# SharperJBCA/COMAPreduce

Measured on AMD Instinct MI355X. Metric: TOD samples x channels / s (L1 -> L2 reduction), higher is better.
Workload: dtype f32 in, f64 accumulate

## Files before the change

### comapreduce_amd/csrc/comap_internal.h

```cpp
#pragma once
#include <hip/hip_runtime.h>
#include <cstdint>
#include <string>
#include <vector>

#include "../../include/comap_hip.h"

struct comap_ctx {
    int device = 0;
    hipStream_t stream = nullptr;
    std::string err;
    void *scratch = nullptr;
    size_t scratch_bytes = 0;
};

#define COMAP_CHECK(ctx, expr)                                                         \
    do {                                                                               \
        hipError_t _e = (expr);                                                        \
        if (_e != hipSuccess) {                                                        \
            (ctx)->err = std::string(#expr) + ": " + hipGetErrorString(_e);            \
            return -2;                                                                 \
        }                                                                              \
    } while (0)

// ... 102 lines not shown
    int32_t wmL = 0;
    size_t wm_smem = 0;
    int32_t *slo = nullptr;
    int32_t *redo = nullptr;
    void *krange = nullptr;
    void *temp = nullptr;
    size_t temp_bytes = 0;
    int64_t numax = 0;
    bool blocksort = true;
    hipEvent_t plan_ev = nullptr;
    hipStream_t alloc_stream = nullptr;
    hipStream_t run_stream = nullptr;
};

int comap_median_plan(comap_ctx *ctx, MedPlan *mp, const std::vector<MedJob> &jobs, int32_t w);
void comap_median_plan_free(MedPlan *mp);
int comap_median_run(comap_ctx *ctx, MedPlan *mp, hipStream_t stream);
inline int comap_median_run(comap_ctx *ctx, MedPlan *mp) { return comap_median_run(ctx, mp, ctx->stream); }
int comap_median_replay(comap_ctx *ctx, const std::vector<MedJob> &jobs, int32_t w, hipStream_t st);

struct comap_l1_plan {
    comap_ctx *ctx = nullptr;
    int32_t F = 0, S = 0, U = 0;
    int64_t T = 0;
    const float *tod = nullptr;
    const double *el = nullptr;
    std::vector<int32_t> units_h;
    int32_t *units = nullptr;
    int32_t *tiles = nullptr;
    int64_t n_tiles = 0;
    int32_t *tiles_b = nullptr;
    int64_t *gaps = nullptr;
    int64_t n_gaps = 0, max_gap = 0;
    static constexpr int kMaxGroups = 4;
    int32_t ngroups = 0;
    int32_t grp_u0[kMaxGroups + 1] = {0};
    int64_t grp_tile0[kMaxGroups + 1] = {0};
    int64_t grpb_tile0[kMaxGroups + 1] = {0};
    MedPlan medg[kMaxGroups];
    hipStream_t side = nullptr;
    hipEvent_t ev_b[kMaxGroups] = {}, ev_m[kMaxGroups] = {};
    double *airmass = nullptr;
    double *unit_sums = nullptr;
    double *mom = nullptr;
    int32_t *nan_count = nullptr;
    bool moments_valid = false;
    bool moments_pending = false;
    bool prefetched = false;
    int32_t *nan_host = nullptr;
    hipEvent_t mom_event = nullptr;
    double *alpha = nullptr;
    double *nf = nullptr;
    double *bsum = nullptr;
    double *mb = nullptr;
    double *mf = nullptr;
    double *ssum = nullptr;
    double *sdm = nullptr;
    double *sgb = nullptr;
    double *pdot = nullptr;
    double *pgate = nullptr;
    int32_t *needc = nullptr;
    bool regress_legacy = false;
    double *gw = nullptr;
    int32_t *gmode = nullptr;
    double *kap = nullptr;
    double *dsum = nullptr;
    double *xreg = nullptr;
    double *dG = nullptr;
    int32_t *rowbad = nullptr;
    int32_t nan_total = 0;
    bool filled = false;
    int64_t *nanpos = nullptr;
    int64_t nanpos_cap = 0;
    int64_t *nanpos_n = nullptr;
// ... 32 lines not shown
```

### comapreduce_amd/csrc/l1_kernels.hip

```cpp
#include "comap_internal.h"

#include <algorithm>
#include <cfloat>
#include <cmath>
#include <cstdlib>
#include <cstring>
#include <type_traits>
#include <utility>

using namespace comap;

#ifndef COMAP_GROUPS
#define COMAP_GROUPS 1
#endif

typedef float f32x4u __attribute__((ext_vector_type(4), aligned(4)));
__device__ __forceinline__ f32x4u ld4(const float *p)
{
    return __builtin_nontemporal_load(reinterpret_cast<const f32x4u *>(p));
}

__device__ __forceinline__ double wave_sum(double v)
{
#pragma unroll
    for (int o = 32; o > 0; o >>= 1) v += __shfl_xor(v, o, 64);
    return v;
}

__device__ __forceinline__ int uniform(int v) { return __builtin_amdgcn_readfirstlane(v); }

__device__ __forceinline__ double block_sum256(double v, double *lds4)
{
    v = wave_sum(v);
    const int wid = threadIdx.x >> 6;
    __syncthreads();
    if ((threadIdx.x & 63) == 0) lds4[wid] = v;
    __syncthreads();
    double t = lds4[0] + lds4[1] + lds4[2] + lds4[3];
    return t;
}

__device__ __forceinline__ bool atmos_channel(int c)
{
    return c >= 10 && c < 1014 && !(c >= 510 && c < 515);
}

__device__ __forceinline__ bool median_channel(int c)
// ... 333 lines not shown
{
    const int64_t i = blockIdx.x * (int64_t)blockDim.x + threadIdx.x;
    if (i >= (int64_t)U * kBC) return;
    const int u = (int)(i / kBC);
    const int bc = (int)(i % kBC);
    const int b = bc / kChannels, c = bc % kChannels;
    const int f = units[4 * u], s = units[4 * u + 1];
    const double *q = ubs + 4 * ((int64_t)u * kBands + b);
    const double n = q[0], sa = q[1], saa = q[2];
    double o = NAN, a = NAN;
    if (atmos_channel(c) && n >= 100.0) {
        const double *src = (sel && sel[(int64_t)u * kBands + b]) ? fs_sel : fs;
        const double sd = src[i], sad = src[UC + i];
        const double det = n * saa - sa * sa;
        o = (saa * sd - sa * sad) / det;
        a = (n * sad - sa * sd) / det;
    }
    double *out = fit + (((int64_t)s * F + f) * kBands + b) * 2 * kChannels;
    out[c] = o;
    out[kChannels + c] = a;
}

__global__ void __launch_bounds__(256) k_coef_b(const int32_t *__restrict__ units, const double *__restrict__ us,
                                                const double *__restrict__ mom, int64_t UC,
                                                const double *__restrict__ fit, int F, const float *__restrict__ med,
                                                double *__restrict__ oa,
                                                double *__restrict__ alpha, double *__restrict__ nf,
                                                double *__restrict__ bsum, int32_t *__restrict__ flag)
{
    __shared__ double red[4];
    const int ub = blockIdx.x;
    const int u = ub / kBands, b = ub % kBands;
    const int n = units[4 * u + 3];
    if (ub == 0 && threadIdx.x == 0) *flag = 0;
    const int fu = units[4 * u], su = units[4 * u + 1];
    const double *fo = fit + (((int64_t)su * F + fu) * kBands + b) * 2 * kChannels;
    const double *q = us + 8 * (int64_t)u;
    const double sv = q[3], svv = q[4], n4 = q[5];
    double beta = 0, gamma = 0, cnt = 0;
    for (int c = threadIdx.x; c < kChannels; c += blockDim.x) {
        const int64_t i = (int64_t)u * kBC + b * kChannels + c;
        const double o = med ? (double)med[i] : fo[c], a = med ? 0.0 : fo[kChannels + c];
        oa[2 * i] = o;
        oa[2 * i + 1] = a;
        double rms = NAN;
        if (n4 > 0 && isfinite(o) && isfinite(a)) {
            const double su = mom[2 * UC + i], suu = mom[3 * UC + i], suv = mom[4 * UC + i];
            const double mean = (su - a * sv) / n4;
            double var = (suu - 2.0 * a * suv + a * a * svv) / n4 - mean * mean;
            var = var < 0.0 ? 0.0 : var;
            rms = sqrt(var) / sqrt(2.0) * sqrt(kDnuTau);
        }
        nf[i] = rms;
        double al = 0.0;
        if (median_channel(c)) {
            al = 1.0 / rms;
            if (isfinite(al) && isfinite(o) && isfinite(a)) {
                beta += al * o;
                gamma += al * a;
                cnt += 1.0;
            } else {
                al = 0.0;
            }
        }
        alpha[i] = al;
    }
    beta = block_sum256(beta, red);
// ... 353 lines not shown
        x1 = y1 / u11;
        x0 = (sym - Smm * x1) / Smf;
    } else {
        const double l = Smf / n, u11 = Smm - l * Smf;
        const double y1 = sym - l * sy;
        x1 = y1 / u11;
        x0 = (sy - Smf * x1) / n;
    }
}

__device__ __forceinline__ bool special_row(bool band_on, int c, double al, int32_t rb)
{
    return band_on && median_channel(c) && al != 0.0 && rb > 0;
}

__device__ __forceinline__ double special_y(double al, double o, double a, double x0, double x1, float d, double At,
                                            double mft)
{
    const double m = ((double)d - (o + a * At)) * al;
    return m - (x0 + mft * x1);
}

__device__ __forceinline__ void special_weights(int c, double tsv, double nf, double g, double y0, double &W,
                                                double &Wo)
{
    W = 1.0 / (tsv * tsv);
    if (tsv == 0.0) W = 0.0;
    if (c < 50 || c >= 974 || c == 512 || (c >= 510 && c < 515)) W = 0.0;
    if (isnan(y0 * nf / g)) W = 0.0;
    Wo = W;
    if (isnan(tsv) || isnan(y0 * tsv)) Wo = 0.0;
}

__global__ void __launch_bounds__(256) k_coef_d(const int32_t *__restrict__ units, const double *__restrict__ us,
                                                const double *__restrict__ mom, int64_t UC,
                                                const double *__restrict__ oa,
                                                const double *__restrict__ alpha, const double *__restrict__ nf,
                                                const double *__restrict__ bsum, const double *__restrict__ ss,
                                                double *__restrict__ sdm, const double *__restrict__ tsys0,
                                                const double *__restrict__ gain0, const double *__restrict__ gw,
                                                const int32_t *__restrict__ gmode, int calibrator,
                                                double *__restrict__ kap, double *__restrict__ dsum,
                                                double *__restrict__ xreg, int phase,
                                                int32_t *__restrict__ flag, int32_t *__restrict__ dlist,
                                                int32_t *__restrict__ dcnt, double *__restrict__ dw,
                                                const int32_t *__restrict__ rowbad, const float *__restrict__ tod,
                                                int64_t T, const double *__restrict__ A,
                                                const double *__restrict__ mf, const int32_t *__restrict__ ynf,
                                                const int32_t *__restrict__ ugate, const double *__restrict__ pd,
                                                double *__restrict__ pg, const int32_t *__restrict__ needc)
{
    __shared__ double red[4];
    __shared__ double s_kap[4][kChannels];
    const int ub = blockIdx.x;
    const int u = ub / kBands, b = ub % kBands;
    const int f = units[4 * u];
    const double *q = us + 8 * (int64_t)u;
    const double n = q[0], SA = q[1];
    const double *bs = bsum + 4 * (int64_t)ub;
    const bool band_on = bs[3] > 0;
    const double *sq = ss + 4 * (int64_t)ub;
    const double Smf = sq[0], Smm = sq[1], SAm = sq[2];
    const int gm = gmode[f];
    const bool gate = n >= 5.0 && !(ugate && ugate[u]);
    const bool gain_called = !calibrator && gate;
    const bool zero = gain_called;
    const bool use_dg = gain_called && gm == 0 && !ynf[u];
    const double det = n * Smm - Smf * Smf;
    const bool fused = phase != 0 && band_on && needc[ub] == 0;
    const bool solve = phase != 0 && !fused;
    double pbad = 0.0, pmag = 0.0;
    double acc[12];
#pragma unroll
    for (int k = 0; k < 12; ++k) acc[k] = 0.0;
    for (int c = threadIdx.x; c < kChannels; c += blockDim.x) {
        const int64_t i = (int64_t)u * kBC + b * kChannels + c;
        const double o = oa[2 * i], a = oa[2 * i + 1];
        const double al = alpha[i];
        const double tsv = tsys0[(int64_t)f * kBC + b * kChannels + c];
        const bool zeroed = zero && (gain_masked(c) || isnan(tsv));
        const bool special = special_row(band_on, c, al, rowbad[i]) && !zeroed;
        double fa = 0, fb = 0, fg = 0, fd = 0, x0 = 0, x1 = 0;
        if (band_on && median_channel(c)) {
            if (al != 0.0) {
                const double sdmi = solve ? sdm[i] : 0.0;
                const double sy = al * (mom[i] - n * o - a * SA);
                const double sym = al * (sdmi - o * Smf - a * SAm);
// ... 166 lines not shown
                const int64_t i = kb + rows[k];
                const double y = special_y(alpha[i], oa[2 * i], oa[2 * i + 1], xreg[2 * i], xreg[2 * i + 1],
                                           tod[(fb + rows[k]) * T + t0 + t], a[t], m[t]);
                inf |= isinf(y);
            }
        if (inf) ugate[u] = 1;
        return;
    }
    const double *ds = dsum + 16 * (int64_t)ub;
    const double SW = ds[10], SWo = ds[11];
    double *to = tod_out + ((int64_t)f * kBands + b) * T + t0;
    double *oo = orig_out + ((int64_t)f * kBands + b) * T + t0;
    for (int t = threadIdx.x; t < n; t += blockDim.x) {
        double sr = 0.0, so = 0.0;
        for (int k = 0; k < nr; ++k) {
            const int c = rows[k];
            const int64_t i = kb + c;
            const double y = special_y(alpha[i], oa[2 * i], oa[2 * i + 1], xreg[2 * i], xreg[2 * i + 1],
                                       tod[(fb + c) * T + t0 + t], a[t], m[t]);
            double r = y * nf[i] / gain0[fb + c];
            if (isnan(r)) r = 0.0;
            sr += rw[k] * r;
            double q = y * tsys0[fb + c];
            if (isnan(q)) q = 0.0;
            so += rwo[k] * q;
        }
        to[t] += sr / SW;
        oo[t] += so / SWo;
    }
}

__global__ void __launch_bounds__(256) k_gain_avg(const float *__restrict__ tod, const double *__restrict__ A,
                                                  const int32_t *__restrict__ units, const int32_t *__restrict__ tiles,
                                                  int64_t T, int64_t UC, const double *__restrict__ kap,
                                                  const double *__restrict__ dsum, const double *__restrict__ mf,
                                                  double *__restrict__ tod_out, double *__restrict__ orig_out,
                                                  double *__restrict__ dG_out, const int32_t *__restrict__ flag)
{
    __shared__ double sg[kBands][kTile];
    if (*flag == 0) return;
    const int b = uniform(threadIdx.x >> 6);
    const int lane = threadIdx.x & 63;
    const int u = tiles[2 * blockIdx.x], toff = tiles[2 * blockIdx.x + 1];
    const int f = units[4 * u], t0 = units[4 * u + 2], n = units[4 * u + 3];
    const int r0 = toff + 4 * lane;
    const float *base = tod + (int64_t)(f * kBands + b) * kChannels * T + t0 + r0;
    const int64_t kb = (int64_t)u * kBC + b * kChannels;
    const double *kg = kap + kb, *kr = kap + UC + kb, *ko = kap + 2 * UC + kb;
    double ag[4 * kJ], ar[4 * kJ], ao[4 * kJ];
#pragma unroll
    for (int i = 0; i < 4 * kJ; ++i) ag[i] = ar[i] = ao[i] = 0.0;
    const int nv0 = n - r0;
#pragma unroll 2
    for (int c = 0; c < kChannels; ++c) {
        const double wg = kg[c], wr = kr[c], wo = ko[c];
        if (wg == 0.0 && wr == 0.0 && wo == 0.0) continue;
        double x[4 * kJ];
        load_groups(base + (int64_t)c * T, nv0, x);
#pragma unroll
        for (int i = 0; i < 4 * kJ; ++i) {
            ag[i] = fma(wg, x[i], ag[i]);
            ar[i] = fma(wr, x[i], ar[i]);
            ao[i] = fma(wo, x[i], ao[i]);
        }
    }
    const double *ds = dsum + 16 * ((int64_t)u * kBands + b);
    const double *a = A + (int64_t)f * T + t0 + r0;
    const double *m = mf + (int64_t)(f * kBands + b) * T + t0 + r0;
    double at[4 * kJ], mt[4 * kJ];
#pragma unroll
    for (int g = 0; g < kJ; ++g)
#pragma unroll
        for (int e = 0; e < 4; ++e) {
            const int i = 4 * g + e, o = 256 * g + e;
            const bool ok = o < nv0;
            at[i] = ok ? a[o] : 0.0;
// ... 12 lines not shown
            const int tl = 256 * g + 4 * lane + e;
            const double dG = sg[0][tl] + sg[1][tl] + sg[2][tl] + sg[3][tl];
            const double sr = ar[i] + ds[3] + at[i] * ds[4] + mt[i] * ds[5];
            const double so = ao[i] + ds[6] + at[i] * ds[7] + mt[i] * ds[8];
            to[o] = (sr - dG * ds[9]) / ds[10];
            oo[o] = so / ds[11];
            if (b == 0) dG_out[(int64_t)f * T + t0 + r0 + o] = dG;
        }
}

__device__ __forceinline__ void scan_weight_band(const double *__restrict__ r, int n, double *__restrict__ wo,
                                                 double *red)
{
    const int np = n / 2;
    double s = 0, cnt = 0;
    for (int k = threadIdx.x; k < np; k += blockDim.x) {
        const double d = r[2 * k + 1] - r[2 * k];
        if (!isnan(d)) { s += d; cnt += 1.0; }
    }
    s = block_sum256(s, red);
    cnt = block_sum256(cnt, red);
    const double mean = s / cnt;
    double v = 0;
    for (int k = threadIdx.x; k < np; k += blockDim.x) {
        const double d = r[2 * k + 1] - r[2 * k];
        if (!isnan(d)) v += (d - mean) * (d - mean);
    }
    v = block_sum256(v, red);
    const double rms = sqrt(v / cnt) / sqrt(2.0);
    const double wt = 1.0 / (rms * rms);
    for (int t = threadIdx.x; t < n; t += blockDim.x) wo[t] = wt;
}

__global__ void __launch_bounds__(256) k_scan_weights(const int32_t *__restrict__ units, int64_t T,
                                                      const double *__restrict__ tod_out, double *__restrict__ w_out)
{
    __shared__ double red[4];
    const int ub = blockIdx.x;
    const int u = ub / kBands, b = ub % kBands;
    const int f = units[4 * u], t0 = units[4 * u + 2], n = units[4 * u + 3];
    const int64_t o = (int64_t)(f * kBands + b) * T + t0;
    scan_weight_band(tod_out + o, n, w_out + o, red);
}

__global__ void __launch_bounds__(256) k_finish(const int32_t *__restrict__ units, const int32_t *__restrict__ tiles,
                                                int64_t T, const double *__restrict__ A,
                                                const double *__restrict__ mf, const double *__restrict__ dsum,
                                                double *__restrict__ tod_out, double *__restrict__ orig_out,
                                                double *__restrict__ dG, const int32_t *__restrict__ flag)
{
    if (*flag != 0) return;
    const int u = tiles[2 * blockIdx.x];
    const int f = units[4 * u], t0 = units[4 * u + 2], n = units[4 * u + 3];
    const double *ds = dsum + 16 * (int64_t)u * kBands;
    for (int k = threadIdx.x; k < kTile; k += 256) {
        const int r = tiles[2 * blockIdx.x + 1] + k;
        if (r >= n) break;
        const int64_t t = t0 + r;
        const double a = A[(int64_t)f * T + t];
        double m[kBands], g = dG[(int64_t)f * T + t];
#pragma unroll
        for (int b = 0; b < kBands; ++b) {
            m[b] = mf[(int64_t)(f * kBands + b) * T + t];
            const double *d = ds + 16 * b;
            g += d[0] + a * d[1] + m[b] * d[2];
        }
        dG[(int64_t)f * T + t] = g;
#pragma unroll
        for (int b = 0; b < kBands; ++b) {
            const double *d = ds + 16 * b;
            const int64_t o = (int64_t)(f * kBands + b) * T + t;
            tod_out[o] = (tod_out[o] + d[3] + a * d[4] + m[b] * d[5] - g * d[9]) / d[10];
            orig_out[o] = (orig_out[o] + d[6] + a * d[7] + m[b] * d[8]) / d[11];
        }
    }
}

__global__ void __launch_bounds__(256) k_zero_gaps(const int64_t *__restrict__ gaps, int64_t T, int F,
                                                   double *__restrict__ tod_out, double *__restrict__ orig_out,
                                                   double *__restrict__ w_out)
{
    const int64_t *g = gaps + 3 * (int64_t)blockIdx.y;
    const int64_t f = g[0], t0 = g[1], n = g[2];
    for (int64_t k = blockIdx.x * (int64_t)blockDim.x + threadIdx.x; k < n; k += (int64_t)gridDim.x * blockDim.x) {
#pragma unroll
        for (int b = 0; b < kBands; ++b) {
            const int64_t o = (f * kBands + b) * T + t0 + k;
            tod_out[o] = 0.0;
            orig_out[o] = 0.0;
// ... 203 lines not shown
        }
    }
    std::vector<int32_t> tiles;
    for (int u = 0; u < p->U; ++u)
        for (int t = 0; t < p->units_h[4 * u + 3]; t += kTile) { tiles.push_back(u); tiles.push_back(t); }
    p->n_tiles = (int64_t)tiles.size() / 2;
    std::vector<int32_t> tiles_b;
    std::vector<int64_t> tub(p->U + 1, 0);
    for (int u = 0; u < p->U; ++u) {
        const int shift = (p->T % 32 == 0) ? (p->units_h[4 * u + 2] & 31) : 0;
        for (int t = -shift; t < p->units_h[4 * u + 3]; t += kTile) { tiles_b.push_back(u); tiles_b.push_back(t); }
        tub[u + 1] = (int64_t)tiles_b.size() / 2;
    }
    std::vector<int64_t> gaps;
    {
        std::vector<std::vector<std::pair<int64_t, int64_t>>> cov(p->F);
        for (int u = 0; u < p->U; ++u)
            cov[p->units_h[4 * u]].push_back({p->units_h[4 * u + 2], p->units_h[4 * u + 2] + p->units_h[4 * u + 3]});
        for (int f = 0; f < p->F; ++f) {
            std::sort(cov[f].begin(), cov[f].end());
            int64_t t = 0;
            for (auto &c : cov[f]) {
                if (c.first > t) { gaps.push_back(f); gaps.push_back(t); gaps.push_back(c.first - t); }
                t = std::max(t, c.second);
            }
            if (t < p->T) { gaps.push_back(f); gaps.push_back(t); gaps.push_back(p->T - t); }
        }
        p->n_gaps = (int64_t)gaps.size() / 3;
        for (int64_t g = 0; g < p->n_gaps; ++g) p->max_gap = std::max(p->max_gap, gaps[3 * g + 2]);
    }
    const int64_t UC = (int64_t)p->U * kBC;
    int rc = 0;
    if (p->n_gaps) rc |= upload(ctx, (void **)&p->gaps, gaps.data(), gaps.size() * 8);
    rc |= dalloc(ctx, &p->flag, 1);
    rc |= dalloc(ctx, &p->dlist, (size_t)p->U * kBC);
    rc |= dalloc(ctx, &p->dcnt, (size_t)p->U * kBands);
    rc |= dalloc(ctx, &p->dw, 4 * (size_t)p->U * kBC);
    if (hipHostMalloc((void **)&p->nan_host, 4, hipHostMallocDefault) != hipSuccess) rc |= 1;
    if (hipEventCreateWithFlags(&p->mom_event, hipEventDisableTiming) != hipSuccess) rc |= 1;
    rc |= upload(ctx, (void **)&p->units, p->units_h.data(), p->units_h.size() * 4);
    rc |= upload(ctx, (void **)&p->tiles, tiles.data(), tiles.size() * 4);
    rc |= upload(ctx, (void **)&p->tiles_b, tiles_b.data(), tiles_b.size() * 4);
    rc |= dalloc(ctx, &p->airmass, (size_t)p->F * p->T);
    rc |= dalloc(ctx, &p->unit_sums, 8 * (size_t)p->U);
    rc |= dalloc(ctx, &p->mom, 5 * (size_t)UC);
    rc |= dalloc(ctx, &p->nan_count, 1);
    rc |= dalloc(ctx, &p->alpha, UC);
    rc |= dalloc(ctx, &p->nf, UC);
    rc |= dalloc(ctx, &p->bsum, 4 * (size_t)p->U * kBands);
    rc |= dalloc(ctx, &p->mb, (size_t)p->F * kBands * p->T);
    rc |= dalloc(ctx, &p->mf, (size_t)p->F * kBands * p->T);
    rc |= dalloc(ctx, &p->ssum, 4 * (size_t)p->U * kBands);
    rc |= dalloc(ctx, &p->sdm, UC);
    rc |= dalloc(ctx, &p->sgb, (size_t)p->F * kBands * p->T);
    rc |= dalloc(ctx, &p->pdot, 4 * (size_t)p->U * kBands);
    rc |= dalloc(ctx, &p->pgate, 2 * (size_t)p->U * kBands);
    rc |= dalloc(ctx, &p->needc, (size_t)p->U * kBands);
    rc |= dalloc(ctx, &p->gw, (size_t)p->F * kBC);
    rc |= dalloc(ctx, &p->gmode, p->F);
    rc |= dalloc(ctx, &p->kap, 3 * (size_t)UC);
    rc |= dalloc(ctx, &p->dsum, 16 * (size_t)p->U * kBands);
    rc |= dalloc(ctx, &p->xreg, 2 * (size_t)UC);
    rc |= dalloc(ctx, &p->dG, (size_t)p->F * p->T);
    rc |= dalloc(ctx, &p->rowbad, UC);
    rc |= dalloc(ctx, &p->ubs, 4 * (size_t)p->U * kBands);
    rc |= dalloc(ctx, &p->fitsum, 2 * (size_t)UC);
    rc |= dalloc(ctx, &p->oa, 2 * (size_t)UC);
    rc |= dalloc(ctx, &p->ynf, (size_t)p->U);
    rc |= dalloc(ctx, &p->ugate, (size_t)p->U);
    if (rc) { delete p; return -2; }
    if (const char *r = getenv("COMAP_L1_REGRESS")) {
        if (!strcmp(r, "legacy")) p->regress_legacy = true;
        else if (strcmp(r, "fused")) { comap_l1_plan_destroy(p); return comap_fail(ctx, -1, "COMAP_L1_REGRESS must be fused or legacy"); }
    }
    int groups = COMAP_GROUPS;
    if (const char *g = getenv("COMAP_GROUPS")) groups = atoi(g);
    p->ngroups = std::max(1, std::min(std::min(groups, comap_l1_plan::kMaxGroups), (int)p->U));
    {
        std::vector<int64_t> tu(p->U + 1, 0);
        for (int u = 0; u < p->U; ++u) tu[u + 1] = tu[u] + (p->units_h[4 * u + 3] + kTile - 1) / kTile;
        for (int g = 0; g <= p->ngroups; ++g) {
            p->grp_u0[g] = (int32_t)((int64_t)p->U * g / p->ngroups);
            p->grp_tile0[g] = tu[p->grp_u0[g]];
            p->grpb_tile0[g] = tub[p->grp_u0[g]];
        }
    }
    int prio = 0;
    if (const char *sp = getenv("COMAP_SIDE_PRIO"); sp && sp[0] == '1') {
        int lo = 0, hi = 0;
        if (hipDeviceGetStreamPriorityRange(&lo, &hi) == hipSuccess) prio = hi;
    }
    bool ok = hipStreamCreateWithPriority(&p->side, hipStreamNonBlocking, prio) == hipSuccess;
    for (int g = 0; g < p->ngroups && ok; ++g)
        ok = hipEventCreateWithFlags(&p->ev_b[g], hipEventDisableTiming) == hipSuccess &&
             hipEventCreateWithFlags(&p->ev_m[g], hipEventDisableTiming) == hipSuccess;
    if (!ok) { comap_l1_plan_destroy(p); return comap_fail(ctx, -2, "side stream / events"); }
    for (int g = 0; g < p->ngroups; ++g) {
        std::vector<MedJob> jobs;
        for (int u = p->grp_u0[g]; u < p->grp_u0[g + 1]; ++u) {
            const int32_t f = p->units_h[4 * u], t0 = p->units_h[4 * u + 2], n = p->units_h[4 * u + 3];
            for (int b = 0; b < kBands; ++b) {
                MedJob j;
                const int64_t off = (int64_t)(f * kBands + b) * p->T + t0;
                j.src = p->mb + off;
                j.dst = p->mf + off;
                j.n = n;
                j.out_lo = n;
                j.out_hi = (n >= 2 * kMedfiltWindow) ? 2 * (int64_t)n : (int64_t)n;
                j.mode = 1;
                j.pad_ = 0;
                j.gate = p->bsum + 4 * ((int64_t)u * kBands + b) + 3;
                jobs.push_back(j);
            }
        }
        rc = comap_median_plan(ctx, &p->medg[g], jobs, kMedfiltWindow);
        if (rc) { comap_l1_plan_destroy(p); return rc; }
    }
    k_airmass<<<2048, 256, 0, ctx->stream>>>(p->el, p->airmass, (int64_t)p->F * p->T);
    COMAP_LAUNCH_CHECK(ctx);
    k_unit_sums<<<p->U, 256, 0, ctx->stream>>>(p->units, p->airmass, p->T, p->unit_sums);
    COMAP_LAUNCH_CHECK(ctx);
    *out = p;
    return 0;
}

extern "C" int comap_l1_plan_destroy(comap_l1_plan *p)
{
    if (!p) return 0;
    COMAP_DEVICE_GUARD(p->ctx);
    if (p->side) (void)hipStreamSynchronize(p->side);
    void *bufs[] = {p->units, p->tiles, p->tiles_b, p->gaps, p->airmass, p->unit_sums, p->mom,
                    p->nan_count, p->alpha, p->nf, p->bsum, p->mb, p->mf, p->ssum, p->sdm, p->gw,
                    p->gmode, p->kap, p->dsum, p->xreg, p->dG, p->rowbad, p->ubs, p->fitsum, p->oa,
                    p->flag, p->dlist, p->dcnt, p->dw, p->nanpos, p->nanpos_n, p->vane_dev,
                    p->sel_pairs, p->sel_voff, p->sel_flag, p->sel_valid, p->ynf, p->ugate, p->sgb, p->pdot,
                    p->pgate, p->needc};
    for (void *b : bufs)
        if (b) (void)hipFree(b);
    for (int g = 0; g < comap_l1_plan::kMaxGroups; ++g) {
        comap_median_plan_free(&p->medg[g]);
        if (p->ev_b[g]) (void)hipEventDestroy(p->ev_b[g]);
        if (p->ev_m[g]) (void)hipEventDestroy(p->ev_m[g]);
    }
    if (p->side) (void)hipStreamDestroy(p->side);
    if (p->nan_host) (void)hipHostFree(p->nan_host);
    if (p->mom_event) (void)hipEventDestroy(p->mom_event);
    if (p->vane_ev) (void)hipEventDestroy(p->vane_ev);
    if (p->pre_a_ev) (void)hipEventDestroy(p->pre_a_ev);
    if (p->vane_done) (void)hipEventDestroy(p->vane_done);
    if (p->vane_pinned) (void)hipHostFree(p->vane_pinned);
    for (hipEvent_t e : p->prof_pool) (void)hipEventDestroy(e);
    delete p;
    return 0;
}

static int launch_moments(comap_l1_plan *p)
{
    comap_ctx *ctx = p->ctx;
    const int64_t UC = (int64_t)p->U * kBC;
    if (!p->pre_a_ev) COMAP_CHECK(ctx, hipEventCreateWithFlags(&p->pre_a_ev, hipEventDisableTiming));
    COMAP_CHECK(ctx, hipEventRecord(p->pre_a_ev, ctx->stream));
    p->pre_a_valid = true;
    COMAP_CHECK(ctx, hipMemsetAsync(p->nan_count, 0, 4, ctx->stream));
    const int64_t grid = (int64_t)p->U * kBands * (kChannels / (4 * kCPW));
    PROF(p, KV_MOMENTS, k_moments<<<grid, 256, 0, ctx->stream>>>(p->tod, p->airmass, p->units, p->T, p->mom, UC,
                                                                     p->nan_count, p->rowbad));
    COMAP_LAUNCH_CHECK(ctx);
    COMAP_CHECK(ctx, hipMemcpyAsync(p->nan_host, p->nan_count, 4, hipMemcpyDeviceToHost, ctx->stream));
    COMAP_CHECK(ctx, hipEventRecord(p->mom_event, ctx->stream));
    p->moments_pending = true;
    p->moments_valid = true;
    return 0;
}

static int wait_moments(comap_l1_plan *p)
{
// ... 182 lines not shown
    int rc = 0;
    if (!p->moments_valid && (rc = run_moments(p))) return rc;
    if ((rc = wait_moments(p))) return rc;
    struct Restore {
        comap_l1_plan *p;
        ~Restore() { (void)restore_nan(p); }
    } restore{p};
    if (p->nan_total > 0 && !p->filled && (rc = fill_nan_rows(p))) return rc;
    const int64_t UC = (int64_t)p->U * kBC;
    const int UB = p->U * kBands;
    hipStream_t st = ctx->stream;
    DevTemps tmp(st);
    float *cmed = nullptr;
    if (calibrator) {
        std::vector<int64_t> ids(UC);
        for (int64_t i = 0; i < UC; ++i) ids[i] = i;
        COMAP_CHECK(ctx, tmp.alloc(&cmed, (size_t)UC));
        if ((rc = unit_row_medians(p, ids, cmed))) return rc;
    }
    if (p->n_gaps) {
        const unsigned gx = (unsigned)std::min<int64_t>(64, (p->max_gap + 255) / 256);
        k_zero_gaps<<<dim3(gx, (unsigned)p->n_gaps), 256, 0, st>>>(p->gaps, p->T, p->F, tod_out, orig_out, w_out);
        COMAP_LAUNCH_CHECK(ctx);
    }
    PROF(p, KV_COEF_B, k_coef_b<<<UB, 256, 0, st>>>(p->units, p->unit_sums, p->mom, UC, fit, p->F, cmed, p->oa,
                                                    p->alpha, p->nf, p->bsum, p->flag));
    COMAP_LAUNCH_CHECK(ctx);
    PROF(p, KV_GAIN_WEIGHTS, k_gain_weights<<<p->F, 1024, 0, st>>>(tsys0, p->gw, p->gmode));
    COMAP_LAUNCH_CHECK(ctx);
    k_unit_flags<<<p->U, 256, 0, st>>>(p->units, p->alpha, p->rowbad, p->bsum, tsys0, p->ynf);
    COMAP_LAUNCH_CHECK(ctx);
    const bool special = p->nan_total > 0;
    const int force_c = (special || p->regress_legacy) ? 1 : 0;
    auto coef_d = [&](int phase, const int32_t *ugate) {
        k_coef_d<<<UB, 256, 0, st>>>(p->units, p->unit_sums, p->mom, UC, p->oa, p->alpha, p->nf, p->bsum, p->ssum,
                                     p->sdm, tsys0, gain0, p->gw, p->gmode, calibrator, p->kap, p->dsum, p->xreg,
                                     phase, p->flag, p->dlist, p->dcnt, p->dw, p->rowbad, p->tod, p->T, p->airmass,
                                     p->mf, p->ynf, ugate, p->pdot, p->pgate, p->needc);
    };
    auto special_rows = [&](int mode) {
        k_special_rows<<<UB, 256, 0, st>>>(mode, p->units, p->tod, p->T, p->airmass, p->mf, p->oa, p->alpha, p->nf,
                                           p->rowbad, p->bsum, p->xreg, tsys0, gain0, p->dsum, calibrator, p->ugate,
                                           tod_out, orig_out);
    };
    PROF(p, KV_COEF_D, coef_d(0, nullptr));
    COMAP_LAUNCH_CHECK(ctx);
    hipStream_t side = p->ngroups > 1 ? p->side : st;
    for (int g = 0; g < p->ngroups; ++g) {
        const int64_t t0 = p->grpb_tile0[g], nt = p->grpb_tile0[g + 1] - t0;
        const int ub0 = p->grp_u0[g] * kBands, nub = (p->grp_u0[g + 1] - p->grp_u0[g]) * kBands;
            PROF(p, KV_BAND_SUMS, k_band_sums<<<kSubB * nt, 256, 0, st>>>(p->tod, p->airmass, p->units, p->tiles_b, t0,
                                                                        p->T, p->dlist, p->dcnt, p->dw, p->bsum,
                                                                        p->mb, tod_out, orig_out, p->dG, p->sgb));
        COMAP_LAUNCH_CHECK(ctx);
        if (side != st) {
            COMAP_CHECK(ctx, hipEventRecord(p->ev_b[g], st));
            COMAP_CHECK(ctx, hipStreamWaitEvent(side, p->ev_b[g], 0));
        }
        PROF_ON(p, KV_MEDIAN, side, rc = comap_median_run(ctx, &p->medg[g], side));
        if (rc) return rc;
        PROF_ON(p, KV_SERIES_SUMS, side, k_series_sums<<<nub, 256, 0, side>>>(ub0, p->units, p->airmass, p->T,
                                                                             p->bsum, p->mf, p->ssum, p->sgb, tod_out,
                                                                             orig_out, p->pgate, force_c, p->pdot,
                                                                             p->needc));
        COMAP_LAUNCH_CHECK(ctx);
        if (side != st) COMAP_CHECK(ctx, hipEventRecord(p->ev_m[g], side));
    }
    for (int g = 0; g < p->ngroups; ++g) {
        const int ub0 = p->grp_u0[g] * kBands, nub = (p->grp_u0[g + 1] - p->grp_u0[g]) * kBands;
        if (side != st) COMAP_CHECK(ctx, hipStreamWaitEvent(st, p->ev_m[g], 0));
        PROF(p, KV_REGRESS, k_regress<<<nub * kRegBlocks, 256, 0, st>>>(ub0, p->tod, p->mf, p->units, p->T, p->bsum,
                                                                       p->dlist, p->dcnt, p->needc, p->sdm));
        COMAP_LAUNCH_CHECK(ctx);
    }
    PROF(p, KV_COEF_D, coef_d(1, nullptr));
    COMAP_LAUNCH_CHECK(ctx);
    if (special) {
        COMAP_CHECK(ctx, hipMemsetAsync(p->ugate, 0, 4 * (size_t)p->U, st));
        special_rows(0);
        COMAP_LAUNCH_CHECK(ctx);
        coef_d(2, p->ugate);
        COMAP_LAUNCH_CHECK(ctx);
        COMAP_CHECK(ctx, hipMemsetAsync(p->flag, 0xff, 4, st));
    }
    PROF(p, KV_GAIN_AVG, k_gain_avg<<<p->n_tiles, 256, 0, st>>>(p->tod, p->airmass, p->units, p->tiles, p->T, UC,
                                                                p->kap, p->dsum, p->mf, tod_out, orig_out, p->dG,
                                                                p->flag));
    COMAP_LAUNCH_CHECK(ctx);
    PROF(p, KV_FINISH, k_finish<<<p->n_tiles, 256, 0, st>>>(p->units, p->tiles, p->T, p->airmass, p->mf, p->dsum,
                                                            tod_out, orig_out, p->dG, p->flag));
    COMAP_LAUNCH_CHECK(ctx);
    if (special) {
        special_rows(1);
        COMAP_LAUNCH_CHECK(ctx);
    }
    PROF(p, KV_SCAN_WEIGHTS, k_scan_weights<<<UB, 256, 0, st>>>(p->units, p->T, tod_out, w_out));
    COMAP_LAUNCH_CHECK(ctx);
    return 0;
}


extern "C" int comap_l1_vane(comap_l1_plan *p, int64_t vstart, int64_t vlen, const int32_t *hot_h,
                             const int64_t *hoff_h, const int32_t *cold_h, const int64_t *coff_h,
                             double t_hot, double *tsys, double *gain)
{
    if (!p || !hoff_h || !coff_h || !tsys || !gain) return -1;
    COMAP_DEVICE_GUARD(p->ctx);
    comap_ctx *ctx = p->ctx;
    const int FB = p->F * kBands;
    if (vstart < 0 || vstart + vlen > p->T) return comap_fail(ctx, -1, "vane event out of range");
    const int64_t nh = hoff_h[FB], nc = coff_h[FB];
    for (int64_t i = 0; i < nh; ++i)
        if (hot_h[i] < 0 || hot_h[i] >= vlen) return comap_fail(ctx, -1, "hot index out of range");
    for (int64_t i = 0; i < nc; ++i)
        if (cold_h[i] < 0 || cold_h[i] >= vlen) return comap_fail(ctx, -1, "cold index out of range");
    const size_t off_c = (size_t)nh * 4, off_ho = (off_c + (size_t)nc * 4 + 15) & ~(size_t)15;
    const size_t off_co = off_ho + (size_t)(FB + 1) * 8, bytes = off_co + (size_t)(FB + 1) * 8;
    hipStream_t st = ctx->stream;
    static const bool use_side = getenv("COMAP_VANE_SIDE") && getenv("COMAP_VANE_SIDE")[0] == '1';
    hipStream_t vs = (use_side && p->side) ? p->side : st;
    if (vs != st) {
        if (!p->pre_a_ev) COMAP_CHECK(ctx, hipEventCreateWithFlags(&p->pre_a_ev, hipEventDisableTiming));
        if (!p->vane_done) COMAP_CHECK(ctx, hipEventCreateWithFlags(&p->vane_done, hipEventDisableTiming));
        if (!p->pre_a_valid) COMAP_CHECK(ctx, hipEventRecord(p->pre_a_ev, st));
        COMAP_CHECK(ctx, hipStreamWaitEvent(vs, p->pre_a_ev, 0));
    }
    if (!p->vane_ev) COMAP_CHECK(ctx, hipEventCreateWithFlags(&p->vane_ev, hipEventDisableTiming));
    else COMAP_CHECK(ctx, hipEventSynchronize(p->vane_ev));
    if (bytes > p->vane_cap) {
// ... 90 lines not shown
```

Baseline: 738.2 billion.

## Auto-select group count and pipeline per-group tail kernels across streams

Raises the maximum number of unit groups and, by default, derives the group count from k_band_sums occupancy and CU count instead of fixing it at one. The per-group tail (coef_d, gain_avg, finish, scan_weights) is split by group so the last group's median can overlap the earlier groups' regression and tail work, and an optional alternating two-stream pipeline is added. The flag becomes per-group. This costs extra launches and events and a host sync guard on error paths, and groups stay at one when the workload is too small for the occupancy test.

```diff
diff --git a/comapreduce_amd/csrc/comap_internal.h b/comapreduce_amd/csrc/comap_internal.h
--- a/comapreduce_amd/csrc/comap_internal.h
+++ b/comapreduce_amd/csrc/comap_internal.h
@@ -158,14 +158,16 @@
     int32_t *tiles_b = nullptr;
     int64_t *gaps = nullptr;
     int64_t n_gaps = 0, max_gap = 0;
-    static constexpr int kMaxGroups = 4;
+    static constexpr int kMaxGroups = 16;
     int32_t ngroups = 0;
+    bool pipe_alt = false;
     int32_t grp_u0[kMaxGroups + 1] = {0};
     int64_t grp_tile0[kMaxGroups + 1] = {0};
     int64_t grpb_tile0[kMaxGroups + 1] = {0};
     MedPlan medg[kMaxGroups];
     hipStream_t side = nullptr;
     hipEvent_t ev_b[kMaxGroups] = {}, ev_m[kMaxGroups] = {};
+    hipEvent_t ev_pre = nullptr, ev_join = nullptr;
     double *airmass = nullptr;
     double *unit_sums = nullptr;
     double *mom = nullptr;
diff --git a/comapreduce_amd/csrc/l1_kernels.hip b/comapreduce_amd/csrc/l1_kernels.hip
--- a/comapreduce_amd/csrc/l1_kernels.hip
+++ b/comapreduce_amd/csrc/l1_kernels.hip
@@ -11,8 +11,9 @@
 using namespace comap;
 
 #ifndef COMAP_GROUPS
-#define COMAP_GROUPS 1
+#define COMAP_GROUPS 0
 #endif
+constexpr int kGroupsAutoMin = 3;
 
 typedef float f32x4u __attribute__((ext_vector_type(4), aligned(4)));
 __device__ __forceinline__ f32x4u ld4(const float *p)
@@ -412,7 +413,7 @@
     const int ub = blockIdx.x;
     const int u = ub / kBands, b = ub % kBands;
     const int n = units[4 * u + 3];
-    if (ub == 0 && threadIdx.x == 0) *flag = 0;
+    if (ub == 0 && threadIdx.x < comap_l1_plan::kMaxGroups) flag[threadIdx.x] = 0;
     const int fu = units[4 * u], su = units[4 * u + 1];
     const double *fo = fit + (((int64_t)su * F + fu) * kBands + b) * 2 * kChannels;
     const double *q = us + 8 * (int64_t)u;
@@ -832,7 +833,7 @@
     if (isnan(tsv) || isnan(y0 * tsv)) Wo = 0.0;
 }
 
-__global__ void __launch_bounds__(256) k_coef_d(const int32_t *__restrict__ units, const double *__restrict__ us,
+__global__ void __launch_bounds__(256) k_coef_d(int ub0, const int32_t *__restrict__ units, const double *__restrict__ us,
                                                 const double *__restrict__ mom, int64_t UC,
                                                 const double *__restrict__ oa,
                                                 const double *__restrict__ alpha, const double *__restrict__ nf,
@@ -852,7 +853,7 @@
 {
     __shared__ double red[4];
     __shared__ double s_kap[4][kChannels];
-    const int ub = blockIdx.x;
+    const int ub = ub0 + blockIdx.x;
     const int u = ub / kBands, b = ub % kBands;
     const int f = units[4 * u];
     const double *q = us + 8 * (int64_t)u;
@@ -1085,7 +1086,7 @@
 
 __global__ void __launch_bounds__(256) k_gain_avg(const float *__restrict__ tod, const double *__restrict__ A,
                                                   const int32_t *__restrict__ units, const int32_t *__restrict__ tiles,
-                                                  int64_t T, int64_t UC, const double *__restrict__ kap,
+                                                  int64_t tile0, int64_t T, int64_t UC, const double *__restrict__ kap,
                                                   const double *__restrict__ dsum, const double *__restrict__ mf,
                                                   double *__restrict__ tod_out, double *__restrict__ orig_out,
                                                   double *__restrict__ dG_out, const int32_t *__restrict__ flag)
@@ -1094,7 +1095,8 @@
     if (*flag == 0) return;
     const int b = uniform(threadIdx.x >> 6);
     const int lane = threadIdx.x & 63;
-    const int u = tiles[2 * blockIdx.x], toff = tiles[2 * blockIdx.x + 1];
+    const int64_t tile = tile0 + blockIdx.x;
+    const int u = tiles[2 * tile], toff = tiles[2 * tile + 1];
     const int f = units[4 * u], t0 = units[4 * u + 2], n = units[4 * u + 3];
     const int r0 = toff + 4 * lane;
     const float *base = tod + (int64_t)(f * kBands + b) * kChannels * T + t0 + r0;
@@ -1173,11 +1175,11 @@
     for (int t = threadIdx.x; t < n; t += blockDim.x) wo[t] = wt;
 }
 
-__global__ void __launch_bounds__(256) k_scan_weights(const int32_t *__restrict__ units, int64_t T,
+__global__ void __launch_bounds__(256) k_scan_weights(int ub0, const int32_t *__restrict__ units, int64_t T,
                                                       const double *__restrict__ tod_out, double *__restrict__ w_out)
 {
     __shared__ double red[4];
-    const int ub = blockIdx.x;
+    const int ub = ub0 + blockIdx.x;
     const int u = ub / kBands, b = ub % kBands;
     const int f = units[4 * u], t0 = units[4 * u + 2], n = units[4 * u + 3];
     const int64_t o = (int64_t)(f * kBands + b) * T + t0;
@@ -1185,17 +1187,18 @@
 }
 
 __global__ void __launch_bounds__(256) k_finish(const int32_t *__restrict__ units, const int32_t *__restrict__ tiles,
-                                                int64_t T, const double *__restrict__ A,
+                                                int64_t tile0, int64_t T, const double *__restrict__ A,
                                                 const double *__restrict__ mf, const double *__restrict__ dsum,
                                                 double *__restrict__ tod_out, double *__restrict__ orig_out,
                                                 double *__restrict__ dG, const int32_t *__restrict__ flag)
 {
     if (*flag != 0) return;
-    const int u = tiles[2 * blockIdx.x];
+    const int64_t tile = tile0 + blockIdx.x;
+    const int u = tiles[2 * tile];
     const int f = units[4 * u], t0 = units[4 * u + 2], n = units[4 * u + 3];
     const double *ds = dsum + 16 * (int64_t)u * kBands;
     for (int k = threadIdx.x; k < kTile; k += 256) {
-        const int r = tiles[2 * blockIdx.x + 1] + k;
+        const int r = tiles[2 * tile + 1] + k;
         if (r >= n) break;
         const int64_t t = t0 + r;
         const double a = A[(int64_t)f * T + t];
@@ -1465,7 +1468,7 @@
     const int64_t UC = (int64_t)p->U * kBC;
     int rc = 0;
     if (p->n_gaps) rc |= upload(ctx, (void **)&p->gaps, gaps.data(), gaps.size() * 8);
-    rc |= dalloc(ctx, &p->flag, 1);
+    rc |= dalloc(ctx, &p->flag, comap_l1_plan::kMaxGroups);
     rc |= dalloc(ctx, &p->dlist, (size_t)p->U * kBC);
     rc |= dalloc(ctx, &p->dcnt, (size_t)p->U * kBands);
     rc |= dalloc(ctx, &p->dw, 4 * (size_t)p->U * kBC);
@@ -1507,8 +1510,20 @@
         else if (strcmp(r, "fused")) { comap_l1_plan_destroy(p); return comap_fail(ctx, -1, "COMAP_L1_REGRESS must be fused or legacy"); }
     }
     int groups = COMAP_GROUPS;
+    if (groups <= 0) {
+        int per_cu = 0, cus = 0;
+        if (hipOccupancyMaxActiveBlocksPerMultiprocessor(&per_cu, k_band_sums, 256, 0) != hipSuccess) per_cu = 0;
+        if (hipDeviceGetAttribute(&cus, hipDeviceAttributeMultiprocessorCount, ctx->device) != hipSuccess) cus = 0;
+        const int64_t resident = (int64_t)per_cu * cus, fill = resident * 7 / 8, blocks = (int64_t)kSubB * tub[p->U];
+        groups = fill > 0 ? (int)std::min<int64_t>(comap_l1_plan::kMaxGroups, (blocks + fill - 1) / fill) : 1;
+        if (groups < kGroupsAutoMin || blocks * 10 < groups * resident * 7) groups = 1;
+    }
     if (const char *g = getenv("COMAP_GROUPS")) groups = atoi(g);
     p->ngroups = std::max(1, std::min(std::min(groups, comap_l1_plan::kMaxGroups), (int)p->U));
+    if (const char *r = getenv("COMAP_L1_PIPE")) {
+        if (!strcmp(r, "alt")) p->pipe_alt = true;
+        else if (strcmp(r, "chain")) { comap_l1_plan_destroy(p); return comap_fail(ctx, -1, "COMAP_L1_PIPE must be chain or alt"); }
+    }
     {
         std::vector<int64_t> tu(p->U + 1, 0);
         for (int u = 0; u < p->U; ++u) tu[u + 1] = tu[u] + (p->units_h[4 * u + 3] + kTile - 1) / kTile;
@@ -1527,6 +1542,8 @@
     for (int g = 0; g < p->ngroups && ok; ++g)
         ok = hipEventCreateWithFlags(&p->ev_b[g], hipEventDisableTiming) == hipSuccess &&
              hipEventCreateWithFlags(&p->ev_m[g], hipEventDisableTiming) == hipSuccess;
+    ok = ok && hipEventCreateWithFlags(&p->ev_pre, hipEventDisableTiming) == hipSuccess &&
+         hipEventCreateWithFlags(&p->ev_join, hipEventDisableTiming) == hipSuccess;
     if (!ok) { comap_l1_plan_destroy(p); return comap_fail(ctx, -2, "side stream / events"); }
     for (int g = 0; g < p->ngroups; ++g) {
         std::vector<MedJob> jobs;
@@ -1575,6 +1592,8 @@
         if (p->ev_b[g]) (void)hipEventDestroy(p->ev_b[g]);
         if (p->ev_m[g]) (void)hipEventDestroy(p->ev_m[g]);
     }
+    if (p->ev_pre) (void)hipEventDestroy(p->ev_pre);
+    if (p->ev_join) (void)hipEventDestroy(p->ev_join);
     if (p->side) (void)hipStreamDestroy(p->side);
     if (p->nan_host) (void)hipHostFree(p->nan_host);
     if (p->mom_event) (void)hipEventDestroy(p->mom_event);
@@ -1823,10 +1842,10 @@
     COMAP_LAUNCH_CHECK(ctx);
     const bool special = p->nan_total > 0;
     const int force_c = (special || p->regress_legacy) ? 1 : 0;
-    auto coef_d = [&](int phase, const int32_t *ugate) {
-        k_coef_d<<<UB, 256, 0, st>>>(p->units, p->unit_sums, p->mom, UC, p->oa, p->alpha, p->nf, p->bsum, p->ssum,
+    auto coef_d = [&](int phase, int ub0, int nub, int32_t *flag, const int32_t *ugate, hipStream_t s) {
+        k_coef_d<<<nub, 256, 0, s>>>(ub0, p->units, p->unit_sums, p->mom, UC, p->oa, p->alpha, p->nf, p->bsum, p->ssum,
                                      p->sdm, tsys0, gain0, p->gw, p->gmode, calibrator, p->kap, p->dsum, p->xreg,
-                                     phase, p->flag, p->dlist, p->dcnt, p->dw, p->rowbad, p->tod, p->T, p->airmass,
+                                     phase, flag, p->dlist, p->dcnt, p->dw, p->rowbad, p->tod, p->T, p->airmass,
                                      p->mf, p->ynf, ugate, p->pdot, p->pgate, p->needc);
     };
     auto special_rows = [&](int mode) {
@@ -1834,58 +1853,115 @@
                                            p->rowbad, p->bsum, p->xreg, tsys0, gain0, p->dsum, calibrator, p->ugate,
                                            tod_out, orig_out);
     };
-    PROF(p, KV_COEF_D, coef_d(0, nullptr));
+    PROF(p, KV_COEF_D, coef_d(0, 0, UB, p->flag, nullptr, st));
     COMAP_LAUNCH_CHECK(ctx);
-    hipStream_t side = p->ngroups > 1 ? p->side : st;
-    for (int g = 0; g < p->ngroups; ++g) {
+    const int G = p->ngroups;
+    auto band_sums = [&](int g, hipStream_t s) -> int {
         const int64_t t0 = p->grpb_tile0[g], nt = p->grpb_tile0[g + 1] - t0;
+        PROF_ON(p, KV_BAND_SUMS, s, k_band_sums<<<kSubB * nt, 256, 0, s>>>(p->tod, p->airmass, p->units, p->tiles_b, t0,
+                                                                          p->T, p->dlist, p->dcnt, p->dw, p->bsum,
+                                                                          p->mb, tod_out, orig_out, p->dG, p->sgb));
+        COMAP_LAUNCH_CHECK(ctx);
+        return 0;
+    };
+    auto median_sums = [&](int g, hipStream_t s) -> int {
         const int ub0 = p->grp_u0[g] * kBands, nub = (p->grp_u0[g + 1] - p->grp_u0[g]) * kBands;
-            PROF(p, KV_BAND_SUMS, k_band_sums<<<kSubB * nt, 256, 0, st>>>(p->tod, p->airmass, p->units, p->tiles_b, t0,
-                                                                        p->T, p->dlist, p->dcnt, p->dw, p->bsum,
-                                                                        p->mb, tod_out, orig_out, p->dG, p->sgb));
+        int r = 0;
+        PROF_ON(p, KV_MEDIAN, s, r = comap_median_run(ctx, &p->medg[g], s));
+        if (r) return r;
+        PROF_ON(p, KV_SERIES_SUMS, s, k_series_sums<<<nub, 256, 0, s>>>(ub0, p->units, p->airmass, p->T, p->bsum, p->mf,
+                                                                       p->ssum, p->sgb, tod_out, orig_out, p->pgate,
+                                                                       force_c, p->pdot, p->needc));
         COMAP_LAUNCH_CHECK(ctx);
+        return 0;
+    };
+    auto regress = [&](int g0, int g1, hipStream_t s) -> int {
+        const int ub0 = p->grp_u0[g0] * kBands, nub = (p->grp_u0[g1] - p->grp_u0[g0]) * kBands;
+        PROF_ON(p, KV_REGRESS, s, k_regress<<<nub * kRegBlocks, 256, 0, s>>>(ub0, p->tod, p->mf, p->units, p->T, p->bsum,
+                                                                            p->dlist, p->dcnt, p->needc, p->sdm));
+        COMAP_LAUNCH_CHECK(ctx);
+        return 0;
+    };
+    auto tail = [&](int g0, int g1, hipStream_t s) -> int {
+        const int ub0 = p->grp_u0[g0] * kBands, nub = (p->grp_u0[g1] - p->grp_u0[g0]) * kBands;
+        const int64_t t0 = p->grp_tile0[g0], nt = p->grp_tile0[g1] - t0;
+        int32_t *flag = p->flag + g0;
+        PROF_ON(p, KV_COEF_D, s, coef_d(1, ub0, nub, flag, nullptr, s));
+        COMAP_LAUNCH_CHECK(ctx);
+        PROF_ON(p, KV_GAIN_AVG, s, k_gain_avg<<<nt, 256, 0, s>>>(p->tod, p->airmass, p->units, p->tiles, t0, p->T, UC,
+                                                                p->kap, p->dsum, p->mf, tod_out, orig_out, p->dG, flag));
+        COMAP_LAUNCH_CHECK(ctx);
+        PROF_ON(p, KV_FINISH, s, k_finish<<<nt, 256, 0, s>>>(p->units, p->tiles, t0, p->T, p->airmass, p->mf, p->dsum,
+                                                            tod_out, orig_out, p->dG, flag));
+        COMAP_LAUNCH_CHECK(ctx);
+        PROF_ON(p, KV_SCAN_WEIGHTS, s, k_scan_weights<<<nub, 256, 0, s>>>(ub0, p->units, p->T, tod_out, w_out));
+        COMAP_LAUNCH_CHECK(ctx);
+        return 0;
+    };
+    struct SideJoin {
+        hipStream_t s;
+        bool armed = false;
+        ~SideJoin() { if (armed) (void)hipStreamSynchronize(s); }
+    } side_join{p->side};
+    if (G > 1 && p->pipe_alt && !special) {
+        COMAP_CHECK(ctx, hipEventRecord(p->ev_pre, st));
+        COMAP_CHECK(ctx, hipStreamWaitEvent(p->side, p->ev_pre, 0));
+        side_join.armed = true;
+        for (int g = 0; g < G; ++g) {
+            hipStream_t s = (g & 1) ? p->side : st;
+            if (g == 1) COMAP_CHECK(ctx, hipStreamWaitEvent(s, p->ev_b[0], 0));
+            if ((rc = band_sums(g, s))) return rc;
+            if (g == 0) COMAP_CHECK(ctx, hipEventRecord(p->ev_b[0], s));
+            if ((rc = median_sums(g, s))) return rc;
+            if ((rc = regress(g, g + 1, s))) return rc;
+            if ((rc = tail(g, g + 1, s))) return rc;
+        }
+        COMAP_CHECK(ctx, hipEventRecord(p->ev_join, p->side));
+        COMAP_CHECK(ctx, hipStreamWaitEvent(st, p->ev_join, 0));
+        side_join.armed = false;
+        return 0;
+    }
+    hipStream_t side = G > 1 ? p->side : st;
+    for (int g = 0; g < G; ++g) {
+        if ((rc = band_sums(g, st))) return rc;
         if (side != st) {
             COMAP_CHECK(ctx, hipEventRecord(p->ev_b[g], st));
             COMAP_CHECK(ctx, hipStreamWaitEvent(side, p->ev_b[g], 0));
-        }
-        PROF_ON(p, KV_MEDIAN, side, rc = comap_median_run(ctx, &p->medg[g], side));
-        if (rc) return rc;
-        PROF_ON(p, KV_SERIES_SUMS, side, k_series_sums<<<nub, 256, 0, side>>>(ub0, p->units, p->airmass, p->T,
-                                                                             p->bsum, p->mf, p->ssum, p->sgb, tod_out,
-                                                                             orig_out, p->pgate, force_c, p->pdot,
-                                                                             p->needc));
-        COMAP_LAUNCH_CHECK(ctx);
+            side_join.armed = true;
+        }
+        if ((rc = median_sums(g, side))) return rc;
         if (side != st) COMAP_CHECK(ctx, hipEventRecord(p->ev_m[g], side));
     }
-    for (int g = 0; g < p->ngroups; ++g) {
-        const int ub0 = p->grp_u0[g] * kBands, nub = (p->grp_u0[g + 1] - p->grp_u0[g]) * kBands;
+    const int gs = (G > 1 && !special) ? G - 1 : G;
+    for (int g = 0; g < gs; ++g)
         if (side != st) COMAP_CHECK(ctx, hipStreamWaitEvent(st, p->ev_m[g], 0));
-        PROF(p, KV_REGRESS, k_regress<<<nub * kRegBlocks, 256, 0, st>>>(ub0, p->tod, p->mf, p->units, p->T, p->bsum,
-                                                                       p->dlist, p->dcnt, p->needc, p->sdm));
-        COMAP_LAUNCH_CHECK(ctx);
-    }
-    PROF(p, KV_COEF_D, coef_d(1, nullptr));
+    if ((rc = regress(0, gs, st))) return rc;
+    if (!special && (rc = tail(0, gs, st))) return rc;
+    if (gs < G) {
+        COMAP_CHECK(ctx, hipStreamWaitEvent(st, p->ev_m[G - 1], 0));
+        if ((rc = regress(G - 1, G, st))) return rc;
+        if ((rc = tail(G - 1, G, st))) return rc;
+    }
+    side_join.armed = false;
+    if (!special) return 0;
+    PROF(p, KV_COEF_D, coef_d(1, 0, UB, p->flag, nullptr, st));
     COMAP_LAUNCH_CHECK(ctx);
-    if (special) {
-        COMAP_CHECK(ctx, hipMemsetAsync(p->ugate, 0, 4 * (size_t)p->U, st));
-        special_rows(0);
-        COMAP_LAUNCH_CHECK(ctx);
-        coef_d(2, p->ugate);
-        COMAP_LAUNCH_CHECK(ctx);
-        COMAP_CHECK(ctx, hipMemsetAsync(p->flag, 0xff, 4, st));
-    }
-    PROF(p, KV_GAIN_AVG, k_gain_avg<<<p->n_tiles, 256, 0, st>>>(p->tod, p->airmass, p->units, p->tiles, p->T, UC,
+    COMAP_CHECK(ctx, hipMemsetAsync(p->ugate, 0, 4 * (size_t)p->U, st));
+    special_rows(0);
+    COMAP_LAUNCH_CHECK(ctx);
+    coef_d(2, 0, UB, p->flag, p->ugate, st);
+    COMAP_LAUNCH_CHECK(ctx);
+    COMAP_CHECK(ctx, hipMemsetAsync(p->flag, 0xff, 4, st));
+    PROF(p, KV_GAIN_AVG, k_gain_avg<<<p->n_tiles, 256, 0, st>>>(p->tod, p->airmass, p->units, p->tiles, 0, p->T, UC,
                                                                 p->kap, p->dsum, p->mf, tod_out, orig_out, p->dG,
                                                                 p->flag));
     COMAP_LAUNCH_CHECK(ctx);
-    PROF(p, KV_FINISH, k_finish<<<p->n_tiles, 256, 0, st>>>(p->units, p->tiles, p->T, p->airmass, p->mf, p->dsum,
+    PROF(p, KV_FINISH, k_finish<<<p->n_tiles, 256, 0, st>>>(p->units, p->tiles, 0, p->T, p->airmass, p->mf, p->dsum,
                                                             tod_out, orig_out, p->dG, p->flag));
     COMAP_LAUNCH_CHECK(ctx);
-    if (special) {
-        special_rows(1);
-        COMAP_LAUNCH_CHECK(ctx);
-    }
-    PROF(p, KV_SCAN_WEIGHTS, k_scan_weights<<<UB, 256, 0, st>>>(p->units, p->T, tod_out, w_out));
+    special_rows(1);
+    COMAP_LAUNCH_CHECK(ctx);
+    PROF(p, KV_SCAN_WEIGHTS, k_scan_weights<<<UB, 256, 0, st>>>(0, p->units, p->T, tod_out, w_out));
     COMAP_LAUNCH_CHECK(ctx);
     return 0;
 }
```

Result: faster. 763.5 billion (median of 6 runs) (+3.4%).
